# 10258392511/InverseProblemWithDiffusionModel

Measured on AMD Instinct MI355X. Metric: ALD reconstructions/sec (128x128 complex, R=40, 4-coil), higher is better.
Workload: dtype f32 (convolutions: operands as two fp16 pieces = 22 significand bits + 2 signs, three fp16 MFMAs per product, fp32 accumulate; every image scaled into fp16's range by an exact power of two from its producer's per-image maxima: any fp32 input, DESIGN.md 4.2); 1 GPU; ACDC-style 128x128 complex SENSE R=40 4-coil ALD reconstruction, NCSNv2Deepest ngf=128 (94.1M params, seeded random init), sigma 348->0.01 x 2311 levels x 3 steps, L2Penalty, denoise; 14 posterior samples = 14 on rank 0 + 13 per further rank (the 105-sample / 8-GPU partition of BASELINE config 3); samples_total=14, samples_this_rank=14, parallelism=sample-sharded x1, hip_graph=True, state_finite=True

## Files before the change

### include/ipdm.h

```cpp
#ifndef IPDM_H
#define IPDM_H

#include <stdint.h>

#ifdef __cplusplus
extern "C" {
#endif

#define IPDM_OK 0
#define IPDM_EINVAL (-1)
#define IPDM_EUNSUPPORTED (-2)

#define IPDM_ACT_NONE 0
#define IPDM_ACT_ELU 1
#define IPDM_ACT_RELU 2
#define IPDM_ACT_LRELU02 3
#define IPDM_ACT_SWISH 4
#define IPDM_ACT_COPY 5

#define IPDM_AMAX_WAYS 8
#define IPDM_AMAX_SLOT 128

#define IPDM_ABI_VERSION 4
int ipdm_abi_version(void);
// ... 68 lines not shown
int ipdm_ald_singlecoil_step_f32(float* x_re, float* x_im, const float* g_re, const float* g_im,
                                 const float* noise_re, const float* noise_im,
                                 float step, float noise_scale, uint64_t seed, int64_t sample_offset, int64_t step_id,
                                 const ipdm_sched_t* dev_sched, const float* y, const uint8_t* mask, int mask_t,
                                 float coef, int mode, float* workspace , int B, int H,
                                 int W, void* stream);

int ipdm_langevin_step_f32(float* x, const float* g, const float* noise, float step, float noise_scale,
                           uint64_t seed, int64_t sample_offset, int64_t step_id, const ipdm_sched_t* dev_sched,
                           int64_t n_samples, int64_t sample_elems, void* stream);

int ipdm_philox_normal_f32(float* out, uint64_t seed, int64_t sample_offset, int64_t step_id, int plane,
                           int64_t n_samples, int64_t sample_elems, void* stream);

int ipdm_philox_block_host(uint64_t seed, int64_t sample, int64_t step_id, int plane, uint32_t quad, uint32_t* out4);


int ipdm_instnorm_plus_coef_f32(const float* x, const float* alpha, const float* gamma, const float* beta,
                                float* coef, int B, int C, int HW,
                                float* amax_bound ,
                                void* stream);
int ipdm_cond_instnorm_plus_coef_f32(const float* x, const float* embed, const int64_t* labels, int num_classes, int bias,
                                     float* coef, int B, int C, int HW, float* amax_bound, void* stream);
int ipdm_affine_act_f32(const float* x, const float* coef, float* y, int B, int C, int HW, int act, void* stream);
int ipdm_act_f32(const float* x, float* y, int64_t n, int act, void* stream);
int ipdm_scale_shift_f32(const float* x, float* y, int64_t n, float a, float b, void* stream);
int ipdm_add_f32(const float* x, const float* y, float* out, int64_t n, void* stream);
int ipdm_div_sigma_f32(const float* x, const float* sigmas, const int64_t* labels, float* out,
                       int B, int64_t sample_elems, void* stream);
int ipdm_conv3x3_thin_supported(int Cin, int Cout, int H, int W);
int ipdm_conv3x3_thin_f32(const float* x, const float* w, const float* bias,
                          const float* coef ,
                          float* out, int B, int Cin, int Cout, int H, int W, void* stream);
int ipdm_maxpool5_f32(const float* x, float* y, int planes, int H, int W, void* stream);
int ipdm_affine_avgpool5_f32(const float* x, const float* coef, float* y, int planes, int H, int W, void* stream);
int ipdm_meanpool2_f32(const float* x, float* y, int planes, int H, int W, void* stream);
int ipdm_bilinear_f32(const float* x, float* out, int planes, int in_h, int in_w, int out_h, int out_w,
                      int accumulate, int act ,
                      int planes_per_image, float* amax_out ,
                      void* stream);
int ipdm_trilinear_f32(const float* x, float* out, int planes, int in_d, int in_h, int in_w, int out_d, int out_h,
                       int out_w, int accumulate, int act, int planes_per_image, float* amax_out, void* stream);

int ipdm_groupnorm_coef_f32(const float* x, const float* weight, const float* bias, float* coef,
                            int B, int C, int HW, int G, float eps,
                            float* plane_amax ,
                            void* stream);
int ipdm_groupnorm_coef_partials_f32(const float* part1, int C1, const float* part2, int C2, int P, const float* weight,
                                     const float* bias, float* coef , int B, int G, float eps, void* stream);
int ipdm_groupnorm_coef_cat_f32(const float* x1, int C1, const float* x2, int C2, const float* weight, const float* bias,
                                float* coef, int B, int HW, int G, float eps, float* plane_amax ,
                                void* stream);
int ipdm_affine_act_cat_f32(const float* x1, int C1, const float* x2, int C2, const float* coef, float* y, int B, int HW,
                            int act, void* stream);
int ipdm_linear_f32(const float* x, const float* W, const float* bias, float* y, int B, int In, int Out,
                    int act, void* stream);
int ipdm_attention_f32(const float* q, const float* k, const float* v, float* out, int B, int C, int N,
                       float scale, void* stream);
int ipdm_axpby_f32(const float* x, const float* y, float* out, int64_t n, float a, float b, void* stream);
int ipdm_sample_axpy2_f32(const float* x, const float* y, const float* z, const float* a, const float* c,
                          float* out, int n_samples, int64_t sample_elems, void* stream);
int ipdm_sample_norm_f32(const float* x, float* norms, int n_samples, int64_t sample_elems, void* stream);

int ipdm_conv_pack_weight_f32(const float* w , float* wt, int Cout, int Cin, int k, void* stream);
int ipdm_conv2d_f32(const float* x, const float* wt, const float* bias, const float* coef, int act,
                    const float* residual, float* out, float* out_act, int act_out,
// ... 137 lines not shown
```

### inverseproblemwithdiffusionmodel_amd/_lib.py

```python
import ctypes
import os

import torch
from ctypes import c_char_p, c_float, c_int, c_int64, c_uint64, c_void_p


class ConvExt(ctypes.Structure):
    _fields_ = [("in_amax", c_void_p), ("bias_bstride", c_int), ("out_scale", c_float), ("res_second", c_int),
                ("out_amax", c_void_p), ("act_amax", c_void_p)]


_HERE = os.path.dirname(os.path.abspath(__file__))
LIB_PATH = os.environ.get("IPDM_LIB") or os.path.join(_HERE, "libipdm.so")

P = c_void_p

SIGNATURES = {
    "ipdm_abi_version": [],
    "ipdm_build_arch": [],
    "ipdm_upfirdn2d_f32": [P, P, P] + [c_int] * 14 + [P],
    "ipdm_fused_bias_act_f32": [P, P, P, P, c_int64, c_int, c_int, c_int, c_int, c_float, c_float, P],
    "ipdm_upfirdn2d_f16": [P, P, P] + [c_int] * 14 + [P],
    "ipdm_upfirdn2d_f64": [P, P, P] + [c_int] * 14 + [P],
    "ipdm_fused_bias_act_f16": [P, P, P, P, c_int64, c_int, c_int, c_int, c_int, c_float, c_float, P],
    "ipdm_fused_bias_act_f64": [P, P, P, P, c_int64, c_int, c_int, c_int, c_int, c_float, c_float, P],
    "ipdm_fft2c_c64": [P, P, c_int, c_int, c_int, c_int, P, P],
    "ipdm_fft2c_workspace_bytes": [c_int, c_int, c_int],
    "ipdm_sense_forward_c64": [P, P, P, c_int, P, c_int, c_int, c_int, c_int, P],
    "ipdm_sense_workspace_bytes": [c_int, c_int, c_int, c_int],
    "ipdm_sense_adjoint_c64": [P, P, P, c_int, c_int, P, P, c_int, c_int, c_int, c_int, P],
    "ipdm_sense_ssos_c64": [P, P, P, c_int, c_int, c_int, c_int, P],
    "ipdm_sense_l2prox_f32": [P, P, P, P, P, c_int, c_float, P, P, P, c_int, c_int, c_int, c_int, P],
    "ipdm_ald_sense_step_f32": [P, P, P, P, P, P, c_float, c_float, c_uint64, c_int64, c_int64, P,
                                P, P, P, c_int, c_float, P, c_int, c_int, c_int, c_int, P],
    "ipdm_singlecoil_prox_f32": [P, P, P, P, c_int, c_float, c_int, P, P, P, c_int, c_int, c_int, P],
    "ipdm_ald_singlecoil_step_f32": [P, P, P, P, P, P, c_float, c_float, c_uint64, c_int64, c_int64, P,
                                     P, P, c_int, c_float, c_int, P, c_int, c_int, c_int, P],
    "ipdm_langevin_step_f32": [P, P, P, c_float, c_float, c_uint64, c_int64, c_int64, P, c_int64, c_int64, P],
    "ipdm_philox_normal_f32": [P, c_uint64, c_int64, c_int64, c_int, c_int64, c_int64, P],
    "ipdm_philox_block_host": [c_uint64, c_int64, c_int64, c_int, ctypes.c_uint32, P],
    "ipdm_instnorm_plus_coef_f32": [P, P, P, P, P, c_int, c_int, c_int, P, P],
    "ipdm_cond_instnorm_plus_coef_f32": [P, P, P, c_int, c_int, P, c_int, c_int, c_int, P, P],
    "ipdm_affine_act_f32": [P, P, P, c_int, c_int, c_int, c_int, P],
    "ipdm_act_f32": [P, P, c_int64, c_int, P],
    "ipdm_scale_shift_f32": [P, P, c_int64, c_float, c_float, P],
    "ipdm_add_f32": [P, P, P, c_int64, P],
    "ipdm_div_sigma_f32": [P, P, P, P, c_int, c_int64, P],
    "ipdm_maxpool5_f32": [P, P, c_int, c_int, c_int, P],
    "ipdm_affine_avgpool5_f32": [P, P, P, c_int, c_int, c_int, P],
    "ipdm_meanpool2_f32": [P, P, c_int, c_int, c_int, P],
    "ipdm_bilinear_f32": [P, P, c_int, c_int, c_int, c_int, c_int, c_int, c_int, c_int, P, P],
    "ipdm_conv3x3_thin_supported": [c_int, c_int, c_int, c_int],
    "ipdm_conv3x3_thin_f32": [P, P, P, P, P, c_int, c_int, c_int, c_int, c_int, P],
    "ipdm_trilinear_f32": [P, P, c_int, c_int, c_int, c_int, c_int, c_int, c_int, c_int, c_int, c_int, P, P],
    "ipdm_groupnorm_coef_f32": [P, P, P, P, c_int, c_int, c_int, c_int, c_float, P, P],
    "ipdm_groupnorm_coef_partials_f32": [P, c_int, P, c_int, c_int, P, P, P, c_int, c_int, c_float, P],
    "ipdm_groupnorm_coef_cat_f32": [P, c_int, P, c_int, P, P, P, c_int, c_int, c_int, c_float, P, P],
    "ipdm_affine_act_cat_f32": [P, c_int, P, c_int, P, P, c_int, c_int, c_int, P],
    "ipdm_linear_f32": [P, P, P, P, c_int, c_int, c_int, c_int, P],
    "ipdm_attention_f32": [P, P, P, P, c_int, c_int, c_int, c_float, P],
    "ipdm_axpby_f32": [P, P, P, c_int64, c_float, c_float, P],
    "ipdm_sample_axpy2_f32": [P, P, P, P, P, P, c_int, c_int64, P],
    "ipdm_sample_norm_f32": [P, P, c_int, c_int64, P],
    "ipdm_conv_pack_weight_f32": [P, P, c_int, c_int, c_int, P],
    "ipdm_conv2d_f32": [P, P, P, P, c_int, P, P, P, c_int] + [c_int] * 8 + [P],
    "ipdm_conv_wino_weight_f32": [P, P, c_int, c_int, P],
    "ipdm_conv2d_wino_supported": [c_int, c_int, c_int, c_int, c_int],
    "ipdm_conv2d_wino_f32": [P, P, P, P, P, P, c_int, c_int, c_int, c_int, c_int, c_int, c_int, P],
    "ipdm_debug_set_stamp_buffer": [P],
    "ipdm_conv3d_f32": [P, P, P, P, c_int, P, P, P, c_int] + [c_int] * 8 + [P],
    "ipdm_maxpool3d5_f32": [P, P, c_int, c_int, c_int, c_int, P],
    "ipdm_temporal_taps_f32": [P, P, c_int, c_int, c_int, c_int, c_int, P],
    "ipdm_conv_bx3_weight_bytes": [c_int, c_int, c_int],
    "ipdm_conv_bx3_pack_weight": [P, P, c_int, c_int, c_int, P],
    "ipdm_conv2d_bx3_f32": [P, P, P, P, c_int, P, P, P, c_int] + [c_int] * 7 + [P, P],
    "ipdm_conv3d_bx3_f32": [P, P, P, P, c_int, P, P, P, c_int] + [c_int] * 8 + [P, P],
    "ipdm_conv_bx3_splitk": [c_int] * 8,
    "ipdm_conv_bx3_splitk_f32": [P, P, P, P, c_int, P, P, P, c_int] + [c_int] * 10 + [P, P, P],
    "ipdm_adam_ascent_f32": [P, P, P, P, c_int64, c_float, c_float, c_float, c_float, c_int, P],
    "ipdm_conv_wino_bx3_weight_bytes": [c_int, c_int],
    "ipdm_conv_wino_bx3_pack_weight": [P, P, c_int, c_int, P],
    "ipdm_conv2d_wino_bx3_supported": [c_int, c_int, c_int, c_int, c_int],
    "ipdm_conv2d_wino_bx3_f32": [P, P, P, P, P, P, c_int, c_int, c_int, c_int, c_int, c_int, c_int, c_int, P, P],
    "ipdm_conv2d_wino_bx3_stats_partials": [c_int, c_int, c_int, c_int, c_int, c_int],
    "ipdm_conv2d_wino_bx3_splitk": [c_int, c_int, c_int, c_int, c_int],
    "ipdm_conv2d_wino_bx3_splitk_f32": [P, P, P, P, P, P, c_int, c_int, c_int, c_int, c_int, c_int, c_int, c_int, P, P, P],
# ... 82 lines not shown
```

### inverseproblemwithdiffusionmodel_amd/csrc/conv_thin.hip

```cpp
#include "ipdm_common.h"

namespace {

template <int CIN>
__global__ __launch_bounds__(256) void conv3x3_fewin_kernel(const float* __restrict__ x, const float* __restrict__ w,
                                                            const float* __restrict__ bias, const float* __restrict__ coef,
                                                            float* __restrict__ out, int B, int Cout, int H, int W,
                                                            int co_blk) {
  const int Q = W >> 2;
  const long long items = (long long)B * H * Q;
  const int co0 = blockIdx.y * co_blk;
  const int co1 = min(Cout, co0 + co_blk);
  for (long long it = (long long)blockIdx.x * 256 + threadIdx.x; it < items; it += (long long)gridDim.x * 256) {
    const int q = (int)(it % Q);
    const long long t = it / Q;
    const int y = (int)(t % H);
    const int b = (int)(t / H);
    float in[CIN][3][6];
#pragma unroll
    for (int ci = 0; ci < CIN; ++ci) {
      float c0 = 0.f, c1 = 1.f, c2 = 0.f;
      if (coef) {
        const float* cf = coef + ((long long)b * CIN + ci) * 3;
        c0 = cf[0]; c1 = cf[1]; c2 = cf[2];
      }
#pragma unroll
      for (int r = 0; r < 3; ++r) {
        const int yy = y + r - 1;
        const bool row_ok = yy >= 0 && yy < H;
        const float* rp = x + (((long long)b * CIN + ci) * H + (row_ok ? yy : 0)) * W + 4 * q;
        const float4 m = *reinterpret_cast<const float4*>(rp);
        const float l = rp[q > 0 ? -1 : 0], rr = rp[q < Q - 1 ? 4 : 3];
        in[ci][r][0] = (row_ok && q > 0) ? (l - c0) * c1 + c2 : 0.f;
        in[ci][r][1] = row_ok ? (m.x - c0) * c1 + c2 : 0.f;
        in[ci][r][2] = row_ok ? (m.y - c0) * c1 + c2 : 0.f;
// ... 96 lines not shown
      for (int j = 0; j < 4; ++j) {
        float v = acc[co][1][j];
        if (up) v += acc[co][0][j];
        if (dn) v += acc[co][2][j];
        o[co][j] = v;
      }
      float left = hl[co][1], right = hr[co][1];
      if (up) { left += hl[co][0]; right += hr[co][0]; }
      if (dn) { left += hl[co][2]; right += hr[co][2]; }
      if (lf) o[co][0] += left;
      if (rt) o[co][3] += right;
    }
    if (grp > 0) {
#pragma unroll
      for (int co = 0; co < COUT; ++co)
#pragma unroll
        for (int j = 0; j < 4; ++j) red[grp - 1][co][j][lane] = o[co][j];
    }
    __syncthreads();
    if (grp == 0 && live) {
#pragma unroll
      for (int co = 0; co < COUT; ++co) {
        const float bv = bias ? bias[co] : 0.f;
        float v[4];
#pragma unroll
        for (int j = 0; j < 4; ++j) v[j] = bv + (((o[co][j] + red[0][co][j][lane]) + red[1][co][j][lane]) + red[2][co][j][lane]);
        *reinterpret_cast<float4*>(out + (((long long)b * COUT + co) * H + y) * W + 4 * q) = make_float4(v[0], v[1], v[2], v[3]);
      }
    }
    __syncthreads();
  }
}

}

extern "C" int ipdm_conv3x3_thin_supported(int Cin, int Cout, int H, int W) {
  return (W % 4 == 0 && H > 0 && ((Cin >= 1 && Cin <= 3 && Cout >= 1) || (Cout >= 1 && Cout <= 3 && Cin >= 1))) ? 1 : 0;
}

extern "C" int ipdm_conv3x3_thin_f32(const float* x, const float* w, const float* bias, const float* coef, float* out, int B,
                                     int Cin, int Cout, int H, int W, void* stream) {
  IPDM_REQUIRE(B >= 0 && Cin > 0 && Cout > 0 && H > 0 && W > 0);
  if (!ipdm_conv3x3_thin_supported(Cin, Cout, H, W)) return IPDM_EUNSUPPORTED;
  if (B == 0) return IPDM_OK;
  IPDM_REQUIRE(x && w && out && x != out);
  IPDM_REQUIRE(((reinterpret_cast<uintptr_t>(x) | reinterpret_cast<uintptr_t>(out)) & 15) == 0);
  hipStream_t s = ipdm_stream(stream);
  const long long items = (long long)B * H * (W / 4);
  const int gx = ipdm_ew_grid(items, 256);
  if (Cin <= 3 && Cin <= Cout) {
    int co_blk = Cout;
    while (co_blk > 8 && (long long)gx * ((Cout + co_blk - 1) / co_blk) < 2048) co_blk = (co_blk + 1) / 2;
    const dim3 grid(gx, (Cout + co_blk - 1) / co_blk);
    if (Cin == 1) hipLaunchKernelGGL(conv3x3_fewin_kernel<1>, grid, dim3(256), 0, s, x, w, bias, coef, out, B, Cout, H, W, co_blk);
    else if (Cin == 2) hipLaunchKernelGGL(conv3x3_fewin_kernel<2>, grid, dim3(256), 0, s, x, w, bias, coef, out, B, Cout, H, W, co_blk);
    else hipLaunchKernelGGL(conv3x3_fewin_kernel<3>, grid, dim3(256), 0, s, x, w, bias, coef, out, B, Cout, H, W, co_blk);
  } else {
    if (coef) return IPDM_EUNSUPPORTED;
    const int Q = W / 4;
    const int gx = ipdm_ew_grid(items, 64);
    const bool shfl = Q <= 64 && 64 % Q == 0;
#define IPDM_FEWOUT(CO)                                                                                                     \
  if (shfl) hipLaunchKernelGGL((conv3x3_fewout_kernel<CO, true>), dim3(gx), dim3(256), 0, s, x, w, bias, out, B, Cin, H, W); \
  else hipLaunchKernelGGL((conv3x3_fewout_kernel<CO, false>), dim3(gx), dim3(256), 0, s, x, w, bias, out, B, Cin, H, W)
    if (Cout == 1) { IPDM_FEWOUT(1); }
    else if (Cout == 2) { IPDM_FEWOUT(2); }
    else { IPDM_FEWOUT(3); }
#undef IPDM_FEWOUT
  }
  return ipdm_launch_status();
}
```

### inverseproblemwithdiffusionmodel_amd/csrc/ipdm_common.h

```cpp
#pragma once
#include <hip/hip_runtime.h>
#include <stdint.h>
#include "ipdm.h"

#define IPDM_WAVE 64

#define IPDM_REQUIRE(cond)          \
  do {                              \
    if (!(cond)) return IPDM_EINVAL; \
  } while (0)

static inline int ipdm_launch_status() {
  hipError_t e = hipGetLastError();
  return e == hipSuccess ? IPDM_OK : (int)e;
}

static inline hipStream_t ipdm_stream(void* s) { return (hipStream_t)s; }

static inline int ipdm_ew_grid(int64_t work_items, int block) {
  int64_t g = (work_items + block - 1) / block;
  if (g > 2048) g = 2048;
  if (g < 1) g = 1;
  return (int)g;
}

__device__ __forceinline__ float ipdm_act(float v, int act) {
  switch (act) {
    case IPDM_ACT_ELU: return v > 0.f ? v : expm1f(v);
    case IPDM_ACT_RELU: return v > 0.f ? v : 0.f;
    case IPDM_ACT_LRELU02: return v > 0.f ? v : 0.2f * v;
    case IPDM_ACT_SWISH: return v / (1.f + expf(-v));
    default: return v;
  }
}

template <int ACT>
__device__ __forceinline__ float ipdm_act_t(float v) {
  if constexpr (ACT == IPDM_ACT_ELU) return v > 0.f ? v : expm1f(v);
  else if constexpr (ACT == IPDM_ACT_RELU) return v > 0.f ? v : 0.f;
  else if constexpr (ACT == IPDM_ACT_LRELU02) return v > 0.f ? v : 0.2f * v;
  else if constexpr (ACT == IPDM_ACT_SWISH) return v / (1.f + expf(-v));
  else return v;
}

__device__ __forceinline__ float ipdm_wave_sum(float v) {
#pragma unroll
  for (int o = 32; o > 0; o >>= 1) v += __shfl_xor(v, o, 64);
  return v;
}
__device__ __forceinline__ double ipdm_wave_sum(double v) {
#pragma unroll
  for (int o = 32; o > 0; o >>= 1) v += __shfl_xor(v, o, 64);
  return v;
}

constexpr int IPDM_AMAX_WAY_STRIDE = 16;

__device__ __forceinline__ float ipdm_wave_max(float v) {
  v = fmaxf(v, __builtin_bit_cast(float, __builtin_amdgcn_update_dpp(0, __builtin_bit_cast(int, v), 0xB1, 0xf, 0xf, false)));
  v = fmaxf(v, __builtin_bit_cast(float, __builtin_amdgcn_update_dpp(0, __builtin_bit_cast(int, v), 0x4E, 0xf, 0xf, false)));
  v = fmaxf(v, __builtin_bit_cast(float, __builtin_amdgcn_update_dpp(0, __builtin_bit_cast(int, v), 0x141, 0xf, 0xf, false)));
  v = fmaxf(v, __builtin_bit_cast(float, __builtin_amdgcn_update_dpp(0, __builtin_bit_cast(int, v), 0x140, 0xf, 0xf, false)));
  v = fmaxf(v, __shfl_xor(v, 16, 64));
  return fmaxf(v, __shfl_xor(v, 32, 64));
}
__device__ __forceinline__ void ipdm_amax_atomic(float* image_slot, int way, float m) {
// ... 77 lines not shown
```

### inverseproblemwithdiffusionmodel_amd/csrc/norm_act.hip

```cpp
#include "ipdm_common.h"

namespace {

template <bool REG>
__global__ __launch_bounds__(256) void plane_stats_kernel(const float* __restrict__ x, float* __restrict__ coef,
                                                          int HW) {
  __shared__ double red[4];
  const float* p = x + (size_t)blockIdx.x * HW;
  const int tid = threadIdx.x, lane = tid & 63, wave = tid >> 6;
  const bool vec = REG || ((HW % 4 == 0) && ((reinterpret_cast<uintptr_t>(p) & 15) == 0));
  float4 keep[16];
  float s = 0.f;
  if constexpr (REG) {
    const int n4 = HW / 4;
#pragma unroll
    for (int k = 0; k < 16; ++k) {
      const int i = tid + k * 256;
      keep[k] = i < n4 ? reinterpret_cast<const float4*>(p)[i] : make_float4(0.f, 0.f, 0.f, 0.f);
    }
#pragma unroll
    for (int k = 0; k < 16; ++k)
      if (tid + k * 256 < n4) s += (keep[k].x + keep[k].y) + (keep[k].z + keep[k].w);
  } else if (vec) {
    for (int i = tid; i < HW / 4; i += 256) {
// ... 148 lines not shown
      const double nn = n + nb, d = mb - mean;
      mean += d * (nb / nn);
      m2 += qb + d * d * (n * nb / nn);
      n = nn;
    }
  }
#pragma unroll
  for (int m = 1; m < 64; m <<= 1) {
    const double nb = __shfl_xor(n, m, 64), mb = __shfl_xor(mean, m, 64), qb = __shfl_xor(m2, m, 64);
    const double nn = n + nb;
    if (nn > 0.0) {
      const double d = mb - mean;
      const double new_mean = (n * mean + nb * mb) / nn;
      m2 = (m2 + qb) + d * d * (n * nb / nn);
      mean = new_mean;
      n = nn;
    }
  }
  if (lane == 0) {
    coef[(size_t)pl * 3 + 0] = (float)mean;
    coef[(size_t)pl * 3 + 1] = 1.0f / sqrtf((float)(m2 / n) + 1e-5f);
  }
}

__global__ __launch_bounds__(256) void affine_act_kernel(const float* x, const float* __restrict__ coef, float* y,
                                                         int HW, int act) {
  const size_t plane = blockIdx.y;
  const float mu = coef[plane * 3], sc = coef[plane * 3 + 1], sh = coef[plane * 3 + 2];
  const float* p = x + plane * HW;
  float* o = y + plane * HW;
  if ((HW & 3) == 0) {
    for (int i = blockIdx.x * 256 + threadIdx.x; i < HW / 4; i += gridDim.x * 256) {
      float4 v = reinterpret_cast<const float4*>(p)[i];
      v.x = ipdm_act((v.x - mu) * sc + sh, act);
      v.y = ipdm_act((v.y - mu) * sc + sh, act);
      v.z = ipdm_act((v.z - mu) * sc + sh, act);
      v.w = ipdm_act((v.w - mu) * sc + sh, act);
      reinterpret_cast<float4*>(o)[i] = v;
    }
  } else {
    for (int i = blockIdx.x * 256 + threadIdx.x; i < HW; i += gridDim.x * 256) o[i] = ipdm_act((p[i] - mu) * sc + sh, act);
  }
}

__global__ __launch_bounds__(256) void affine_act_cat_kernel(const float* x1, int C1, const float* x2, int C2,
                                                             const float* __restrict__ coef, float* y, int HW, int act) {
  const size_t plane = blockIdx.y;
  const int Ct = C1 + C2;
  const size_t b = plane / Ct;
  const int c = (int)(plane % Ct);
  const float mu = coef[plane * 3], sc = coef[plane * 3 + 1], sh = coef[plane * 3 + 2];
  const float* p = c < C1 ? x1 + (b * C1 + c) * HW : x2 + (b * C2 + (c - C1)) * HW;
  float* o = y + plane * HW;
  if ((HW & 3) == 0) {
    for (int i = blockIdx.x * 256 + threadIdx.x; i < HW / 4; i += gridDim.x * 256) {
      float4 v = reinterpret_cast<const float4*>(p)[i];
      v.x = ipdm_act((v.x - mu) * sc + sh, act);
      v.y = ipdm_act((v.y - mu) * sc + sh, act);
      v.z = ipdm_act((v.z - mu) * sc + sh, act);
      v.w = ipdm_act((v.w - mu) * sc + sh, act);
      reinterpret_cast<float4*>(o)[i] = v;
    }
  } else {
    for (int i = blockIdx.x * 256 + threadIdx.x; i < HW; i += gridDim.x * 256) o[i] = ipdm_act((p[i] - mu) * sc + sh, act);
  }
}

template <typename F>
__global__ __launch_bounds__(256) void ew1_kernel(const float* x, float* y, int64_t n, F f) {
  const int64_t nv = n / 4;
  const bool vec = ((reinterpret_cast<uintptr_t>(x) | reinterpret_cast<uintptr_t>(y)) & 15) == 0;
  const int64_t tid = (int64_t)blockIdx.x * 256 + threadIdx.x, stride = (int64_t)gridDim.x * 256;
  if (vec) {
    for (int64_t i = tid; i < nv; i += stride) {
// ... 568 lines not shown
```

### inverseproblemwithdiffusionmodel_amd/ncsn/models/layers.py

```python
import os
from functools import partial

import torch
import torch.nn as nn

from ... import ops, _lib
from .normalization import InstanceNorm2dPlus, ConditionalInstanceNorm2dPlus, get_normalization


class _Act:

    def __init__(self, name):
        self.name = name
        self.code = ops.ACT_CODES[name]

    def __call__(self, x):
        return ops.act(x, self.code)


USE_WINOGRAD = os.environ.get("IPDM_WINOGRAD", "1") != "0"
FUSE_POOL = os.environ.get("IPDM_FUSE_POOL", "1") != "0"


def get_act(config):
# ... 23 lines not shown
        self.in_planes, self.out_planes, self.kernel_size, self.dilation = in_planes, out_planes, kernel_size, dilation
        self.ndim = ndim
        self.full_range = full_range
        self.weight = nn.Parameter(torch.empty(out_planes, in_planes, *([kernel_size] * ndim)))
        self.bias = nn.Parameter(torch.empty(out_planes)) if bias else None
        bound = 1.0 / (in_planes * kernel_size ** ndim) ** 0.5
        nn.init.uniform_(self.weight, -bound, bound)
        if bias:
            nn.init.uniform_(self.bias, -bound, bound)
        self._cache = ops.PackedWeightCache()

    def _cached(self, kind, build):
        return self._cache.get(self.weight, kind, build)

    def packed_wino(self):
        return self._cached("wino_f32", ops.conv_wino_weight)

    def packed_wino_bx3(self):
        return self._cached("wino_" + ops.CONV_IMPL, ops.conv_wino_split_weight)

    def packed_wino1d(self):
        return self._cached("wino1d", ops.conv_wino1d_weight)

    def fuses_input(self, x, coef):
        return (ops.WINO1D_FIN and USE_WINOGRAD and ops.split_impl() and self.ndim == 2 and self.kernel_size == 3 and x.dim() == 4
                and x.data_ptr() % 16 == 0 and (not ops.dynamic_range() or getattr(coef, "_ipdm_amax_bound", None) is not None)
                and ops.wino1d_pays(self.in_planes, self.out_planes, x.shape[2], x.shape[3], self.dilation))

    def packed(self):
        if self.full_range and ops.CONV_IMPL == "hx2":
            return self._cached("direct_bx3", lambda w: ops.conv_weight(w, impl="bx3"))
        return self._cached("direct_" + ops.CONV_IMPL, ops.conv_weight)

    def forward(self, x, coef=None, act=ops.ACT_NONE, residual=None, out=None, act_out=ops.ACT_NONE, raw=True,
                want_stats=False, in_amax=None, feeds_conv=True, res_second=False):
        bias = None if self.bias is None else self.bias.data
        dyn = ops.dynamic_range()
        produce = dyn and feeds_conv
        if in_amax is None and dyn and coef is None and act == ops.ACT_NONE:
            in_amax = ops.in_amax_for(x)
        if coef is not None and act == ops.ACT_ELU and out is None and self.fuses_input(x, coef):
            return ops.conv2d_wino_bx3(x, self.packed_wino1d(), bias, residual, act_out=act_out, raw=raw, want_stats=want_stats,
                                       in_amax=getattr(coef, "_ipdm_amax_bound", None) if dyn else None, want_amax=produce,
                                       res_second=res_second, coef=coef, act=act)
        if (self.ndim == 2 and self.kernel_size == 3 and self.dilation == 1 and act == ops.ACT_NONE
                and residual is None and out is None and act_out == ops.ACT_NONE and raw and x.dim() == 4
                and (self.in_planes <= 3 or (self.out_planes <= 3 and coef is None))
                and ops.conv3x3_thin_ok(self.in_planes, self.out_planes, x.shape[2], x.shape[3])):
            return ops.conv3x3_thin(x, self.weight.data, bias, coef)
        if (USE_WINOGRAD and ops.CONV_IMPL == "f32" and self.ndim == 2 and self.kernel_size == 3 and coef is None and act == ops.ACT_NONE
                and out is None
                and ops.conv_wino_supported(self.in_planes, self.out_planes, x.shape[2], x.shape[3], self.dilation)):
            return ops.conv2d_wino(x, self.packed_wino(), bias, residual, act_out=act_out, raw=raw,
                                   dilation=self.dilation)
        if (USE_WINOGRAD and ops.split_impl() and self.ndim == 2 and self.kernel_size == 3 and coef is None
                and act == ops.ACT_NONE and out is None and ops.wino_bx3_pays(self.in_planes, self.out_planes, x.shape[2],
                                                                              x.shape[3], self.dilation)):
            one_d = (x.data_ptr() % 16 == 0 and act_out in (ops.ACT_NONE, ops.ACT_ELU, ops.ACT_COPY)
                     and (ops.WINO1D_STATS or not (want_stats and raw and ops.USE_STATS_EPILOGUE))
                     and ops.wino1d_pays(self.in_planes, self.out_planes, x.shape[2], x.shape[3], self.dilation))
            return ops.conv2d_wino_bx3(x, self.packed_wino1d() if one_d else self.packed_wino_bx3(), bias, residual,
                                       act_out=act_out, raw=raw, dilation=self.dilation, want_stats=want_stats, in_amax=in_amax,
                                       want_amax=produce, res_second=res_second)
        if (self.ndim == 3 and self.kernel_size == 3 and self.dilation == 1 and coef is None and act == ops.ACT_NONE and out is None
                and x.dim() == 5 and x.data_ptr() % 16 == 0 and act_out in (ops.ACT_NONE, ops.ACT_ELU, ops.ACT_COPY)
                and ops.wino1d_vol_pays(self.in_planes, self.out_planes, x.shape[2], x.shape[3], x.shape[4])):
            return ops.conv3d(x, self._cached("wino1d_vol", ops.conv_wino1d_weight3d), bias, residual=residual, act_out=act_out,
                              raw=raw, in_amax=in_amax, want_amax=produce, res_second=res_second)
        if self.ndim == 3:
            return ops.conv3d(x, self.packed(), bias, coef, act, residual, self.dilation, act_out=act_out, raw=raw,
                              in_amax=in_amax, want_amax=produce, res_second=res_second)
        return ops.conv2d(x, self.packed(), bias, coef, act, residual, self.dilation, out=out, act_out=act_out, raw=raw,
                          in_amax=in_amax, want_amax=produce, res_second=res_second)
# ... 426 lines not shown
```

### inverseproblemwithdiffusionmodel_amd/ncsn/models/ncsn.py

```python
import torch
import torch.nn as nn

from .layers import ConditionalResidualBlock, CondRefineBlock, Conv2d, get_act
from .normalization import get_normalization
from ... import ops


class _NCSNBase(nn.Module):
    def __init__(self, config):
        super().__init__()
        if config.model.spec_norm:
            raise NotImplementedError("spec_norm is unused by every shipped config")
        self.logit_transform = config.data.logit_transform
        self.rescaled = config.data.rescaled
        self.norm = get_normalization(config, conditional=True)
        self.ngf = config.model.ngf
        self.num_classes = config.model.num_classes
        self.act = get_act(config)
        self.config = config
        ngf, ch = self.ngf, config.data.channels
        self.begin_conv = Conv2d(ch, ngf, 3, full_range=True)
        self._in_coef = {}

    def _block(self, cin, cout, resample=None, dilation=None, adjust_padding=False):
        return ConditionalResidualBlock(cin, cout, self.num_classes, resample=resample, act=self.act, normalization=self.norm,
                                        adjust_padding=adjust_padding, dilation=dilation)

    def _stage(self, cin, cout, resample=None, dilation=None, adjust_padding=False):
        return nn.ModuleList([self._block(cin, cout, resample, dilation, adjust_padding), self._block(cout, cout, None, dilation)])

    def _refine(self, in_planes, features, start=False, end=False):
        return CondRefineBlock(in_planes, features, self.num_classes, self.norm, act=self.act, start=start, end=end)

    @staticmethod
    def _compute_cond_module(module, x, y, feeds_conv):
        n = len(module)
        for i, m in enumerate(module):
            x = m(x, y, feeds_conv=feeds_conv and i == n - 1)
        return x

    def _begin(self, x):
        if not x.is_cuda:
            raise RuntimeError("score network: expected GPU tensors (no CPU fallback in this build)")
        x = x.contiguous().float()
        if not self.logit_transform and not self.rescaled:
            key = (x.shape[0], x.shape[1], str(x.device))
            if key not in self._in_coef:
                self._in_coef[key] = torch.tensor([0.5, 2.0, 0.0], device=x.device).repeat(x.shape[0], x.shape[1], 1)
            return self.begin_conv(x, self._in_coef[key])
        return self.begin_conv(x)

    def _end(self, output, y):
        return self.end_conv(self.normalizer(output, y, self.act.code))

    def forward(self, x, y):
        y = y.long()
        with ops.amax_scope():
            return self._forward(x, y)


class NCSN(_NCSNBase):
    def __init__(self, config):
        super().__init__(config)
        ngf, ch = self.ngf, config.data.channels
        self.normalizer = self.norm(ngf, self.num_classes)
        self.end_conv = Conv2d(ngf, ch, 3)
        self.res1 = self._stage(ngf, ngf)
        self.res2 = self._stage(ngf, 2 * ngf, 'down')
        self.res3 = self._stage(2 * ngf, 2 * ngf, 'down', dilation=2)
        self.res4 = self._stage(2 * ngf, 2 * ngf, 'down', dilation=4, adjust_padding=config.data.image_size == 28)
        self.refine1 = self._refine([2 * ngf], 2 * ngf, start=True)
        self.refine2 = self._refine([2 * ngf, 2 * ngf], 2 * ngf)
        self.refine3 = self._refine([2 * ngf, 2 * ngf], ngf)
        self.refine4 = self._refine([ngf, ngf], ngf, end=True)

    def _forward(self, x, y):
        output = self._begin(x)
        layer1 = self._compute_cond_module(self.res1, output, y, True)
        layer2 = self._compute_cond_module(self.res2, layer1, y, True)
        layer3 = self._compute_cond_module(self.res3, layer2, y, True)
        layer4 = self._compute_cond_module(self.res4, layer3, y, False)
        ref1 = self.refine1([layer4], y, layer4.shape[2:])
        ref2 = self.refine2([layer3, ref1], y, layer3.shape[2:])
        ref3 = self.refine3([layer2, ref2], y, layer2.shape[2:])
        output = self.refine4([layer1, ref3], y, layer1.shape[2:])
# ... 34 lines not shown
```

### inverseproblemwithdiffusionmodel_amd/ncsn/models/ncsnv2.py

```python
import torch
import torch.nn as nn

from . import get_sigmas
from .layers import ResidualBlock, RefineBlock, Conv2d, get_act, get_normalization
from ... import ops


class _NCSNv2Base(nn.Module):
    def __init__(self, config):
        super().__init__()
        self.logit_transform = config.data.logit_transform
        self.rescaled = config.data.rescaled
        self.norm = get_normalization(config, conditional=False)
        self.ngf = config.model.ngf
        self.num_classes = config.model.num_classes
        self.act = get_act(config)
        self.register_buffer('sigmas', get_sigmas(config))
        self.config = config
        self._in_coef = {}

    def _compute_cond_module(self, module, x):
        n = len(module)
        for i, m in enumerate(module):
            x = m(x, want_act=(i == n - 1))
        return x

    def _stage(self, cin, cout, resample=None, dilation=None):
        kw = dict(act=self.act, normalization=self.norm)
        if dilation is not None:
            kw["dilation"] = dilation
        return nn.ModuleList([ResidualBlock(cin, cout, resample=resample, **kw),
                              ResidualBlock(cout, cout, resample=None, **kw)])

    def _begin(self, x):
        if not x.is_cuda:
            raise RuntimeError("score network: expected GPU tensors (no CPU fallback in this build)")
        x = x.contiguous().float()
        if not self.logit_transform and not self.rescaled:
            key = (x.shape[0], x.shape[1], str(x.device))
            if key not in self._in_coef:
                self._in_coef[key] = torch.tensor([0.5, 2.0, 0.0], device=x.device).repeat(x.shape[0], x.shape[1], 1)
            return self.begin_conv(x, self._in_coef[key])
        return self.begin_conv(x)

    def _end(self, output, x, y):
        output = self.end_conv(self.normalizer(output, self.act.code))
        sig = self.sigmas if self.sigmas.dtype == torch.float32 else self.sigmas.to(torch.float32)
        return ops.div_sigma(output, sig, y.to(torch.int64))

    @staticmethod
    def _refine(block, pairs, shape, want_act=True):
        return block([p[0] for p in pairs], shape, [p[1] for p in pairs], want_act=want_act)


class NCSNv2Deepest(_NCSNv2Base):
    def __init__(self, config):
        super().__init__(config)
        ngf, ch = self.ngf, config.data.channels
        self.begin_conv = Conv2d(ch, ngf, 3, full_range=True)
        self.normalizer = self.norm(ngf)
        self.end_conv = Conv2d(ngf, ch, 3)
        self.res1 = self._stage(ngf, ngf)
        self.res2 = self._stage(ngf, 2 * ngf, 'down')
        self.res3 = self._stage(2 * ngf, 2 * ngf, 'down')
        self.res31 = self._stage(2 * ngf, 2 * ngf, 'down')
        self.res4 = self._stage(2 * ngf, 4 * ngf, 'down', dilation=2)
        self.res5 = self._stage(4 * ngf, 4 * ngf, 'down', dilation=4)
        self.refine1 = RefineBlock([4 * ngf], 4 * ngf, act=self.act, start=True)
        self.refine2 = RefineBlock([4 * ngf, 4 * ngf], 2 * ngf, act=self.act)
        self.refine3 = RefineBlock([2 * ngf, 2 * ngf], 2 * ngf, act=self.act)
        self.refine31 = RefineBlock([2 * ngf, 2 * ngf], 2 * ngf, act=self.act)
        self.refine4 = RefineBlock([2 * ngf, 2 * ngf], ngf, act=self.act)
        self.refine5 = RefineBlock([ngf, ngf], ngf, act=self.act, end=True)

    def forward(self, x, y):
        with ops.amax_scope():
            return self._forward(x, y)

    def _forward(self, x, y):
# ... 85 lines not shown
```

### inverseproblemwithdiffusionmodel_amd/ops.py

```python
import ctypes
import os

import torch

from . import _lib
from ._lib import call, P

ACT_NONE, ACT_ELU, ACT_RELU, ACT_LRELU02, ACT_SWISH = 0, 1, 2, 3, 4
ACT_COPY = 5
CONV_TRACE = None

ACT_CODES = {"none": ACT_NONE, None: ACT_NONE, "elu": ACT_ELU, "relu": ACT_RELU, "lrelu": ACT_LRELU02,
             "swish": ACT_SWISH}


def _gpu(t, dtype=None, name="tensor"):
    if not isinstance(t, torch.Tensor) or not t.is_cuda:
        raise RuntimeError(f"ipdm: {name} must be a GPU tensor (the HIP path has no CPU fallback); got "
                           f"{getattr(t, 'device', type(t))}")
    if dtype is not None and t.dtype != dtype:
        raise TypeError(f"ipdm: {name} must be {dtype}, got {t.dtype}")
    return t if t.is_contiguous() else t.contiguous()


# ... 869 lines not shown
    call("ipdm_conv2d_f32", _ptr(x), _ptr(wt), _ptr(bias), _ptr(coef), act, _ptr(residual), _ptr(out), _ptr(out_act),
         act_out, B, Cin, Cout, H, W, k, dilation, int(bool(pool2)), _stream())
    _written(out)
    if CONV_TRACE is not None:
        e1.record()
        CONV_TRACE.append(dict(B=B, Cin=Cin, Cout=Cout, H=H, W=W, k=k, dil=dilation, res=residual is not None,
                               n_out=int(raw) + int(want_act), e0=e0, e1=e1))
    return (out, out_act) if want_act else out


USE_THIN_CONV = os.environ.get("IPDM_THIN_CONV", "1") != "0"


def conv3x3_thin_ok(Cin, Cout, H, W):
    return USE_THIN_CONV and bool(_lib.lib.ipdm_conv3x3_thin_supported(int(Cin), int(Cout), int(H), int(W)))


def conv3x3_thin(x, weight, bias=None, coef=None):
    x = _gpu(x, torch.float32, "x")
    weight = _gpu(weight, torch.float32, "weight")
    B, Cin, H, W = x.shape
    Cout = weight.shape[0]
    if tuple(weight.shape) != (Cout, Cin, 3, 3):
        raise ValueError(f"conv3x3_thin: weight {tuple(weight.shape)} does not match input channels {Cin}")
    out = torch.empty((B, Cout, H, W), dtype=torch.float32, device=x.device)
    if CONV_TRACE is not None:
        e0, e1 = torch.cuda.Event(enable_timing=True), torch.cuda.Event(enable_timing=True)
        e0.record()
    if coef is not None:
        coef = _gpu(coef, torch.float32, "coef")
        if tuple(coef.shape) != (B, Cin, 3):
            raise ValueError(f"conv3x3_thin: coef {tuple(coef.shape)} != {(B, Cin, 3)}")
    call("ipdm_conv3x3_thin_f32", _ptr(x), _ptr(weight), _ptr(bias), _ptr(coef), _ptr(out), B, Cin, Cout, H, W, _stream())
    if CONV_TRACE is not None:
        e1.record()
        CONV_TRACE.append(dict(B=B, Cin=Cin, Cout=Cout, H=H, W=W, k=3, dil=1, res=False, n_out=1, e0=e0, e1=e1, thin=True))
    return out


CONV_IMPL = os.environ.get("IPDM_CONV_IMPL", "hx2")
SPLIT_IMPLS = ("hx2", "bx3")
if CONV_IMPL not in SPLIT_IMPLS + ("f32",):
    raise ValueError(f"IPDM_CONV_IMPL={CONV_IMPL!r}: expected 'hx2', 'bx3' or 'f32'")


def split_impl():
    return CONV_IMPL in SPLIT_IMPLS


def impl_unbounded():
    env = os.environ.get("IPDM_CONV_IMPL_UNBOUNDED")
    if env:
        if env not in SPLIT_IMPLS + ("f32",):
            raise ValueError(f"IPDM_CONV_IMPL_UNBOUNDED={env!r}")
        return env
    return CONV_IMPL


def unbounded_amax():
    return True if impl_unbounded() == "hx2" else None


class PackedWeightCache:

    def __init__(self):
        self._entries = {}
# ... 381 lines not shown
```

Baseline: 0.1268 reconstructions/s.

## Fuse end-norm activation into multi-row few-output conv3x3 kernel

Adds a new few-output-channel 3x3 conv kernel that computes several output rows per thread, reusing each loaded input row across vertical taps. The model's final normalizer affine plus activation is applied inside the conv while it loads its input, so the separate normalized activation tensor is never written or read back. Plain thin few-output convs are also routed to the new kernel, with default rows=4 for Cout=1 and 2 otherwise. The costs are higher register pressure from the large per-thread accumulator arrays and a shared-memory reduction across channel groups.

```diff
diff --git a/include/ipdm.h b/include/ipdm.h
--- a/include/ipdm.h
+++ b/include/ipdm.h
@@ -124,6 +124,8 @@
 int ipdm_conv3x3_thin_f32(const float* x, const float* w, const float* bias,
                           const float* coef ,
                           float* out, int B, int Cin, int Cout, int H, int W, void* stream);
+int ipdm_conv3x3_fewout_f32(const float* x, const float* w, const float* bias, const float* coef, int act, float* out,
+                            int B, int Cin, int Cout, int H, int W, int rows, void* stream);
 int ipdm_maxpool5_f32(const float* x, float* y, int planes, int H, int W, void* stream);
 int ipdm_affine_avgpool5_f32(const float* x, const float* coef, float* y, int planes, int H, int W, void* stream);
 int ipdm_meanpool2_f32(const float* x, float* y, int planes, int H, int W, void* stream);
diff --git a/inverseproblemwithdiffusionmodel_amd/_lib.py b/inverseproblemwithdiffusionmodel_amd/_lib.py
--- a/inverseproblemwithdiffusionmodel_amd/_lib.py
+++ b/inverseproblemwithdiffusionmodel_amd/_lib.py
@@ -52,6 +52,7 @@
     "ipdm_bilinear_f32": [P, P, c_int, c_int, c_int, c_int, c_int, c_int, c_int, c_int, P, P],
     "ipdm_conv3x3_thin_supported": [c_int, c_int, c_int, c_int],
     "ipdm_conv3x3_thin_f32": [P, P, P, P, P, c_int, c_int, c_int, c_int, c_int, P],
+    "ipdm_conv3x3_fewout_f32": [P, P, P, P, c_int, P, c_int, c_int, c_int, c_int, c_int, c_int, P],
     "ipdm_trilinear_f32": [P, P, c_int, c_int, c_int, c_int, c_int, c_int, c_int, c_int, c_int, c_int, P, P],
     "ipdm_groupnorm_coef_f32": [P, P, P, P, c_int, c_int, c_int, c_int, c_float, P, P],
     "ipdm_groupnorm_coef_partials_f32": [P, c_int, P, c_int, c_int, P, P, P, c_int, c_int, c_float, P],
diff --git a/inverseproblemwithdiffusionmodel_amd/csrc/conv_thin.hip b/inverseproblemwithdiffusionmodel_amd/csrc/conv_thin.hip
--- a/inverseproblemwithdiffusionmodel_amd/csrc/conv_thin.hip
+++ b/inverseproblemwithdiffusionmodel_amd/csrc/conv_thin.hip
@@ -1,6 +1,8 @@
 #include "ipdm_common.h"
 
 namespace {
+
+constexpr int IPDM_FEWOUT_ROWS_1 = 4;
 
 template <int CIN>
 __global__ __launch_bounds__(256) void conv3x3_fewin_kernel(const float* __restrict__ x, const float* __restrict__ w,
@@ -163,10 +165,228 @@
   }
 }
 
+template <int COUT, int R, bool SHFL, int FUSE>
+__global__ __launch_bounds__(256) void conv3x3_fewout_rows_kernel(const float* __restrict__ x, const float* __restrict__ w,
+                                                                  const float* __restrict__ bias, const float* __restrict__ coef,
+                                                                  int act, float* __restrict__ out, int B, int Cin, int H, int W) {
+  __shared__ float red[3][COUT][R][4][64];
+  constexpr int U = R <= 4 ? 4 : 2;
+  const int Q = W >> 2;
+  const int S = (H + R - 1) / R;
+  const long long items = (long long)B * S * Q;
+  const long long HW = (long long)H * W;
+  const int lane = threadIdx.x & 63, grp = threadIdx.x >> 6;
+  for (long long it0 = (long long)blockIdx.x * 64; it0 < items; it0 += (long long)gridDim.x * 64) {
+    const long long it = it0 + lane < items ? it0 + lane : items - 1;
+    const bool live = it0 + lane < items;
+    const int q = (int)(it % Q);
+    const long long t = it / Q;
+    const int y0 = (int)(t % S) * R;
+    const int b = (int)(t / S);
+    float acc[COUT][R][3][4], hl[COUT][R][3], hr[COUT][R][3];
+#pragma unroll
+    for (int co = 0; co < COUT; ++co)
+#pragma unroll
+      for (int i = 0; i < R; ++i)
+#pragma unroll
+        for (int r = 0; r < 3; ++r) {
+          hl[co][i][r] = 0.f; hr[co][i][r] = 0.f;
+#pragma unroll
+          for (int j = 0; j < 4; ++j) acc[co][i][r][j] = 0.f;
+        }
+    const bool lf = q > 0, rt = q < Q - 1;
+    int ro[R + 2];
+#pragma unroll
+    for (int k = 0; k < R + 2; ++k) ro[k] = min(max(y0 - 1 + k, 0), H - 1) * W;
+    const float* base = x + (long long)b * Cin * HW + 4 * q;
+    const float* cbase = FUSE ? coef + (long long)b * Cin * 3 : nullptr;
+    auto norm_act = [&](float t, const float (&c)[3]) {
+      t = ipdm_affine(t, c[0], c[1], c[2]);
+      if constexpr (FUSE == 2) {
+        float a = t > 0.f ? 0.f : t;
+        asm("" : "+v"(a));
+        const float e = expm1f(a);
+        return t > 0.f ? t : e;
+      } else {
+        return ipdm_act(t, act);
+      }
+    };
+    for (int ci0 = grp; ci0 < Cin; ci0 += 4 * U) {
+      float4 m[U][R + 2];
+      [[maybe_unused]] float el[U][R + 2], er[U][R + 2], cf[U][3];
+#pragma unroll
+      for (int u = 0; u < U; ++u) {
+        const int ci = min(ci0 + 4 * u, Cin - 1);
+        const float* cp = base + ci * HW;
+#pragma unroll
+        for (int k = 0; k < R + 2; ++k) {
+          const float* rp = cp + ro[k];
+          m[u][k] = *reinterpret_cast<const float4*>(rp);
+          if constexpr (!SHFL) {
+            el[u][k] = rp[lf ? -1 : 0];
+            er[u][k] = rp[rt ? 4 : 3];
+          }
+        }
+        if constexpr (FUSE) {
+          cf[u][0] = cbase[ci * 3]; cf[u][1] = cbase[ci * 3 + 1]; cf[u][2] = cbase[ci * 3 + 2];
+        }
+      }
+#pragma unroll
+      for (int u = 0; u < U; ++u) {
+        const int ci = ci0 + 4 * u;
+        if (ci >= Cin) break;
+#pragma unroll
+        for (int k = 0; k < R + 2; ++k) {
+          float4 v = m[u][k];
+          if constexpr (FUSE) {
+            v.x = norm_act(v.x, cf[u]);
+            v.y = norm_act(v.y, cf[u]);
+            v.z = norm_act(v.z, cf[u]);
+            v.w = norm_act(v.w, cf[u]);
+          }
+          float l, rr;
+          if constexpr (SHFL) {
+            l = __shfl_up(v.w, 1, 64);
+            rr = __shfl_down(v.x, 1, 64);
+          } else {
+            l = el[u][k];
+            rr = er[u][k];
+            if constexpr (FUSE) {
+              l = norm_act(l, cf[u]);
+              rr = norm_act(rr, cf[u]);
+            }
+          }
+#pragma unroll
+          for (int r = 0; r < 3; ++r) {
+            const int i = k - r;
+            if (i < 0 || i >= R) continue;
+#pragma unroll
+            for (int co = 0; co < COUT; ++co) {
+              const float* wp = w + ((long long)co * Cin + ci) * 9 + r * 3;
+              const float w0 = wp[0], w1 = wp[1], w2 = wp[2];
+              hl[co][i][r] = fmaf(w0, l, hl[co][i][r]);
+              acc[co][i][r][0] = fmaf(w1, v.x, acc[co][i][r][0]);
+              acc[co][i][r][0] = fmaf(w2, v.y, acc[co][i][r][0]);
+              acc[co][i][r][1] = fmaf(w0, v.x, acc[co][i][r][1]);
+              acc[co][i][r][1] = fmaf(w1, v.y, acc[co][i][r][1]);
+              acc[co][i][r][1] = fmaf(w2, v.z, acc[co][i][r][1]);
+              acc[co][i][r][2] = fmaf(w0, v.y, acc[co][i][r][2]);
+              acc[co][i][r][2] = fmaf(w1, v.z, acc[co][i][r][2]);
+              acc[co][i][r][2] = fmaf(w2, v.w, acc[co][i][r][2]);
+              acc[co][i][r][3] = fmaf(w0, v.z, acc[co][i][r][3]);
+              acc[co][i][r][3] = fmaf(w1, v.w, acc[co][i][r][3]);
+              hr[co][i][r] = fmaf(w2, rr, hr[co][i][r]);
+            }
+          }
+        }
+      }
+    }
+    float o[COUT][R][4];
+#pragma unroll
+    for (int co = 0; co < COUT; ++co)
+#pragma unroll
+      for (int i = 0; i < R; ++i) {
+        const bool up = y0 + i > 0, dn = y0 + i < H - 1;
+#pragma unroll
+        for (int j = 0; j < 4; ++j) {
+          float v = acc[co][i][1][j];
+          if (up) v += acc[co][i][0][j];
+          if (dn) v += acc[co][i][2][j];
+          o[co][i][j] = v;
+        }
+        float left = hl[co][i][1], right = hr[co][i][1];
+        if (up) { left += hl[co][i][0]; right += hr[co][i][0]; }
+        if (dn) { left += hl[co][i][2]; right += hr[co][i][2]; }
+        if (lf) o[co][i][0] += left;
+        if (rt) o[co][i][3] += right;
+      }
+    if (grp > 0) {
+#pragma unroll
+      for (int co = 0; co < COUT; ++co)
+#pragma unroll
+        for (int i = 0; i < R; ++i)
+#pragma unroll
+          for (int j = 0; j < 4; ++j) red[grp - 1][co][i][j][lane] = o[co][i][j];
+    }
+    __syncthreads();
+    if (grp == 0 && live) {
+#pragma unroll
+      for (int co = 0; co < COUT; ++co) {
+        const float bv = bias ? bias[co] : 0.f;
+#pragma unroll
+        for (int i = 0; i < R; ++i) {
+          if (y0 + i >= H) break;
+          float v[4];
+#pragma unroll
+          for (int j = 0; j < 4; ++j)
+            v[j] = bv + (((o[co][i][j] + red[0][co][i][j][lane]) + red[1][co][i][j][lane]) + red[2][co][i][j][lane]);
+          *reinterpret_cast<float4*>(out + (((long long)b * COUT + co) * H + y0 + i) * W + 4 * q) = make_float4(v[0], v[1], v[2], v[3]);
+        }
+      }
+    }
+    __syncthreads();
+  }
+}
+
 }
 
 extern "C" int ipdm_conv3x3_thin_supported(int Cin, int Cout, int H, int W) {
   return (W % 4 == 0 && H > 0 && ((Cin >= 1 && Cin <= 3 && Cout >= 1) || (Cout >= 1 && Cout <= 3 && Cin >= 1))) ? 1 : 0;
+}
+
+static int fewout_default_rows(int Cout) { return Cout == 1 ? IPDM_FEWOUT_ROWS_1 : 2; }
+
+extern "C" int ipdm_conv3x3_fewout_f32(const float* x, const float* w, const float* bias, const float* coef, int act, float* out,
+                                       int B, int Cin, int Cout, int H, int W, int rows, void* stream) {
+  IPDM_REQUIRE(B >= 0 && Cin > 0 && Cout >= 1 && Cout <= 3 && H > 0 && W > 0 && W % 4 == 0);
+  IPDM_REQUIRE(rows == 0 || rows == 1 || rows == 2 || ((rows == 4 || rows == 8) && Cout == 1));
+  IPDM_REQUIRE(act >= IPDM_ACT_NONE && act <= IPDM_ACT_SWISH);
+  if (rows == 1 && coef) return IPDM_EUNSUPPORTED;
+  if (coef && act == IPDM_ACT_SWISH) return IPDM_EUNSUPPORTED;
+  if (B == 0) return IPDM_OK;
+  IPDM_REQUIRE(x && w && out && x != out);
+  IPDM_REQUIRE(((reinterpret_cast<uintptr_t>(x) | reinterpret_cast<uintptr_t>(out)) & 15) == 0);
+  hipStream_t s = ipdm_stream(stream);
+  const int Q = W / 4;
+  const bool shfl = Q <= 64 && 64 % Q == 0;
+  if (rows == 0) rows = fewout_default_rows(Cout);
+  if (rows == 1) {
+    const int gx = ipdm_ew_grid((long long)B * H * Q, 64);
+#define IPDM_FEWOUT(CO)                                                                                                     \
+  if (shfl) hipLaunchKernelGGL((conv3x3_fewout_kernel<CO, true>), dim3(gx), dim3(256), 0, s, x, w, bias, out, B, Cin, H, W); \
+  else hipLaunchKernelGGL((conv3x3_fewout_kernel<CO, false>), dim3(gx), dim3(256), 0, s, x, w, bias, out, B, Cin, H, W)
+    if (Cout == 1) { IPDM_FEWOUT(1); }
+    else if (Cout == 2) { IPDM_FEWOUT(2); }
+    else { IPDM_FEWOUT(3); }
+#undef IPDM_FEWOUT
+    return ipdm_launch_status();
+  }
+  const int gx = ipdm_ew_grid((long long)B * ((H + rows - 1) / rows) * Q, 64);
+#define IPDM_FEWOUT_ROWS_F(CO, R, SH, FU)                                                                                   \
+  hipLaunchKernelGGL((conv3x3_fewout_rows_kernel<CO, R, SH, FU>), dim3(gx), dim3(256), 0, s, x, w, bias, coef, act, out, B, \
+                     Cin, H, W)
+#define IPDM_FEWOUT_ROWS(CO, R)                                                                                              \
+  do {                                                                                                                       \
+    if (shfl && fuse == 2) IPDM_FEWOUT_ROWS_F(CO, R, true, 2);                                                               \
+    else if (shfl && fuse == 1) IPDM_FEWOUT_ROWS_F(CO, R, true, 1);                                                          \
+    else if (shfl) IPDM_FEWOUT_ROWS_F(CO, R, true, 0);                                                                       \
+    else if (fuse == 2) IPDM_FEWOUT_ROWS_F(CO, R, false, 2);                                                                 \
+    else if (fuse == 1) IPDM_FEWOUT_ROWS_F(CO, R, false, 1);                                                                 \
+    else IPDM_FEWOUT_ROWS_F(CO, R, false, 0);                                                                                \
+  } while (0)
+  const int fuse = !coef ? 0 : act == IPDM_ACT_ELU ? 2 : 1;
+  if (Cout == 1) {
+    if (rows == 2) IPDM_FEWOUT_ROWS(1, 2);
+    else if (rows == 4) IPDM_FEWOUT_ROWS(1, 4);
+    else IPDM_FEWOUT_ROWS(1, 8);
+  } else if (Cout == 2) {
+    IPDM_FEWOUT_ROWS(2, 2);
+  } else {
+    IPDM_FEWOUT_ROWS(3, 2);
+  }
+#undef IPDM_FEWOUT_ROWS
+#undef IPDM_FEWOUT_ROWS_F
+  return ipdm_launch_status();
 }
 
 extern "C" int ipdm_conv3x3_thin_f32(const float* x, const float* w, const float* bias, const float* coef, float* out, int B,
@@ -188,16 +408,7 @@
     else hipLaunchKernelGGL(conv3x3_fewin_kernel<3>, grid, dim3(256), 0, s, x, w, bias, coef, out, B, Cout, H, W, co_blk);
   } else {
     if (coef) return IPDM_EUNSUPPORTED;
-    const int Q = W / 4;
-    const int gx = ipdm_ew_grid(items, 64);
-    const bool shfl = Q <= 64 && 64 % Q == 0;
-#define IPDM_FEWOUT(CO)                                                                                                     \
-  if (shfl) hipLaunchKernelGGL((conv3x3_fewout_kernel<CO, true>), dim3(gx), dim3(256), 0, s, x, w, bias, out, B, Cin, H, W); \
-  else hipLaunchKernelGGL((conv3x3_fewout_kernel<CO, false>), dim3(gx), dim3(256), 0, s, x, w, bias, out, B, Cin, H, W)
-    if (Cout == 1) { IPDM_FEWOUT(1); }
-    else if (Cout == 2) { IPDM_FEWOUT(2); }
-    else { IPDM_FEWOUT(3); }
-#undef IPDM_FEWOUT
+    return ipdm_conv3x3_fewout_f32(x, w, bias, nullptr, IPDM_ACT_NONE, out, B, Cin, Cout, H, W, 0, stream);
   }
   return ipdm_launch_status();
 }
diff --git a/inverseproblemwithdiffusionmodel_amd/csrc/ipdm_common.h b/inverseproblemwithdiffusionmodel_amd/csrc/ipdm_common.h
--- a/inverseproblemwithdiffusionmodel_amd/csrc/ipdm_common.h
+++ b/inverseproblemwithdiffusionmodel_amd/csrc/ipdm_common.h
@@ -32,6 +32,12 @@
     case IPDM_ACT_SWISH: return v / (1.f + expf(-v));
     default: return v;
   }
+}
+
+__device__ __forceinline__ float ipdm_affine(float v, float mu, float sc, float sh) {
+  float p = (v - mu) * sc;
+  asm("" : "+v"(p));
+  return p + sh;
 }
 
 template <int ACT>
diff --git a/inverseproblemwithdiffusionmodel_amd/csrc/norm_act.hip b/inverseproblemwithdiffusionmodel_amd/csrc/norm_act.hip
--- a/inverseproblemwithdiffusionmodel_amd/csrc/norm_act.hip
+++ b/inverseproblemwithdiffusionmodel_amd/csrc/norm_act.hip
@@ -204,14 +204,14 @@
   if ((HW & 3) == 0) {
     for (int i = blockIdx.x * 256 + threadIdx.x; i < HW / 4; i += gridDim.x * 256) {
       float4 v = reinterpret_cast<const float4*>(p)[i];
-      v.x = ipdm_act((v.x - mu) * sc + sh, act);
-      v.y = ipdm_act((v.y - mu) * sc + sh, act);
-      v.z = ipdm_act((v.z - mu) * sc + sh, act);
-      v.w = ipdm_act((v.w - mu) * sc + sh, act);
+      v.x = ipdm_act(ipdm_affine(v.x, mu, sc, sh), act);
+      v.y = ipdm_act(ipdm_affine(v.y, mu, sc, sh), act);
+      v.z = ipdm_act(ipdm_affine(v.z, mu, sc, sh), act);
+      v.w = ipdm_act(ipdm_affine(v.w, mu, sc, sh), act);
       reinterpret_cast<float4*>(o)[i] = v;
     }
   } else {
-    for (int i = blockIdx.x * 256 + threadIdx.x; i < HW; i += gridDim.x * 256) o[i] = ipdm_act((p[i] - mu) * sc + sh, act);
+    for (int i = blockIdx.x * 256 + threadIdx.x; i < HW; i += gridDim.x * 256) o[i] = ipdm_act(ipdm_affine(p[i], mu, sc, sh), act);
   }
 }
 
diff --git a/inverseproblemwithdiffusionmodel_amd/ncsn/models/layers.py b/inverseproblemwithdiffusionmodel_amd/ncsn/models/layers.py
--- a/inverseproblemwithdiffusionmodel_amd/ncsn/models/layers.py
+++ b/inverseproblemwithdiffusionmodel_amd/ncsn/models/layers.py
@@ -79,6 +79,11 @@
             return self._cached("direct_bx3", lambda w: ops.conv_weight(w, impl="bx3"))
         return self._cached("direct_" + ops.CONV_IMPL, ops.conv_weight)
 
+    def streams_fewout(self, x, act=ops.ACT_NONE):
+        return (act in ops.FEWOUT_FUSED_ACTS and self.ndim == 2 and self.kernel_size == 3 and self.dilation == 1 and x.dim() == 4
+                and self.in_planes > 3 and self.out_planes <= 3
+                and ops.conv3x3_thin_ok(self.in_planes, self.out_planes, x.shape[2], x.shape[3]))
+
     def forward(self, x, coef=None, act=ops.ACT_NONE, residual=None, out=None, act_out=ops.ACT_NONE, raw=True,
                 want_stats=False, in_amax=None, feeds_conv=True, res_second=False):
         bias = None if self.bias is None else self.bias.data
@@ -86,6 +91,9 @@
         produce = dyn and feeds_conv
         if in_amax is None and dyn and coef is None and act == ops.ACT_NONE:
             in_amax = ops.in_amax_for(x)
+        if (coef is not None and residual is None and out is None and act_out == ops.ACT_NONE and raw
+                and self.streams_fewout(x, act)):
+            return ops.conv3x3_fewout(x, self.weight.data, bias, coef, act)
         if coef is not None and act == ops.ACT_ELU and out is None and self.fuses_input(x, coef):
             return ops.conv2d_wino_bx3(x, self.packed_wino1d(), bias, residual, act_out=act_out, raw=raw, want_stats=want_stats,
                                        in_amax=getattr(coef, "_ipdm_amax_bound", None) if dyn else None, want_amax=produce,
diff --git a/inverseproblemwithdiffusionmodel_amd/ncsn/models/ncsn.py b/inverseproblemwithdiffusionmodel_amd/ncsn/models/ncsn.py
--- a/inverseproblemwithdiffusionmodel_amd/ncsn/models/ncsn.py
+++ b/inverseproblemwithdiffusionmodel_amd/ncsn/models/ncsn.py
@@ -51,6 +51,8 @@
         return self.begin_conv(x)
 
     def _end(self, output, y):
+        if self.end_conv.streams_fewout(output, self.act.code):
+            return self.end_conv(output, coef=self.normalizer.coef(output, y), act=self.act.code)
         return self.end_conv(self.normalizer(output, y, self.act.code))
 
     def forward(self, x, y):
diff --git a/inverseproblemwithdiffusionmodel_amd/ncsn/models/ncsnv2.py b/inverseproblemwithdiffusionmodel_amd/ncsn/models/ncsnv2.py
--- a/inverseproblemwithdiffusionmodel_amd/ncsn/models/ncsnv2.py
+++ b/inverseproblemwithdiffusionmodel_amd/ncsn/models/ncsnv2.py
@@ -44,7 +44,10 @@
         return self.begin_conv(x)
 
     def _end(self, output, x, y):
-        output = self.end_conv(self.normalizer(output, self.act.code))
+        if self.end_conv.streams_fewout(output, self.act.code):
+            output = self.end_conv(output, coef=self.normalizer.coef(output), act=self.act.code)
+        else:
+            output = self.end_conv(self.normalizer(output, self.act.code))
         sig = self.sigmas if self.sigmas.dtype == torch.float32 else self.sigmas.to(torch.float32)
         return ops.div_sigma(output, sig, y.to(torch.int64))
 
diff --git a/inverseproblemwithdiffusionmodel_amd/ops.py b/inverseproblemwithdiffusionmodel_amd/ops.py
--- a/inverseproblemwithdiffusionmodel_amd/ops.py
+++ b/inverseproblemwithdiffusionmodel_amd/ops.py
@@ -925,6 +925,32 @@
         if tuple(coef.shape) != (B, Cin, 3):
             raise ValueError(f"conv3x3_thin: coef {tuple(coef.shape)} != {(B, Cin, 3)}")
     call("ipdm_conv3x3_thin_f32", _ptr(x), _ptr(weight), _ptr(bias), _ptr(coef), _ptr(out), B, Cin, Cout, H, W, _stream())
+    if CONV_TRACE is not None:
+        e1.record()
+        CONV_TRACE.append(dict(B=B, Cin=Cin, Cout=Cout, H=H, W=W, k=3, dil=1, res=False, n_out=1, e0=e0, e1=e1, thin=True))
+    return out
+
+
+FEWOUT_FUSED_ACTS = (ACT_NONE, ACT_ELU, ACT_RELU, ACT_LRELU02)
+
+
+def conv3x3_fewout(x, weight, bias=None, coef=None, act=ACT_NONE, rows=0):
+    x = _gpu(x, torch.float32, "x")
+    weight = _gpu(weight, torch.float32, "weight")
+    B, Cin, H, W = x.shape
+    Cout = weight.shape[0]
+    if tuple(weight.shape) != (Cout, Cin, 3, 3):
+        raise ValueError(f"conv3x3_fewout: weight {tuple(weight.shape)} does not match input channels {Cin}")
+    if coef is not None:
+        coef = _gpu(coef, torch.float32, "coef")
+        if tuple(coef.shape) != (B, Cin, 3):
+            raise ValueError(f"conv3x3_fewout: coef {tuple(coef.shape)} != {(B, Cin, 3)}")
+    out = torch.empty((B, Cout, H, W), dtype=torch.float32, device=x.device)
+    if CONV_TRACE is not None:
+        e0, e1 = torch.cuda.Event(enable_timing=True), torch.cuda.Event(enable_timing=True)
+        e0.record()
+    call("ipdm_conv3x3_fewout_f32", _ptr(x), _ptr(weight), _ptr(bias), _ptr(coef), int(act) if coef is not None else ACT_NONE,
+         _ptr(out), B, Cin, Cout, H, W, int(rows), _stream())
     if CONV_TRACE is not None:
         e1.record()
         CONV_TRACE.append(dict(B=B, Cin=Cin, Cout=Cout, H=H, W=W, k=3, dil=1, res=False, n_out=1, e0=e0, e1=e1, thin=True))
```

After: 0.1276 reconstructions/s, median of 6. No clear change (+0.6%).
